# megvii-research/OccDepth

Measured on AMD Instinct MI355X. Metric: frames/sec forward, SemanticKITTI stereo->256x256x32 voxels, higher is better.
Workload: dtype f32 storage and accumulate; matrix arithmetic as 3x bf16 split (hi + mid + lo of both operands, six v_mfma_f32_32x32x16_bf16 per K step; error vs float64 tested within 1.5x of the exact-fp32 kernels', measured 0.8-1.1x) in the head convolutions (K2s3), the small-volume 3x3x3 convolutions and transpo

## Files before the change

include/occdepth_amd.h:

```cpp
#ifndef OCCDEPTH_AMD_H
#define OCCDEPTH_AMD_H

#include <stdint.h>

#ifdef __cplusplus
extern "C" {
#endif

#define OCCD_OK 0
#define OCCD_EINVAL (-1)
#define OCCD_ELAUNCH (-2)
#define OCCD_ENOMEM (-3)

#define OCCD_MAX_VIEWS 4
#define OCCD_MAX_SCALES 4

#define OCCD_ACT_NONE 0
#define OCCD_ACT_RELU 1
#define OCCD_ACT_SIGMOID 2
#define OCCD_ACT_RELU_PRE 3

#define OCCD_ABI_VERSION 22
int occd_abi_version(void);
const char* occd_strerror(int code);
// ... 153 lines not shown
    const double* cam_E;
    const double* cam_k;
    double voxel_size;
    float origin[3];
    int32_t img_w, img_h;
    occd_flosp_args frustum;
    const float* ida;
} occd_lift_proj_args;
int occd_lift_proj_fwd(const occd_lift_proj_args* a, void* stream);

typedef struct occd_lift_bwd_args {
    occd_lift_args fwd;
    const float* gout;
    float* gfeat[OCCD_MAX_SCALES][OCCD_MAX_VIEWS];
    float* gdepth;
} occd_lift_bwd_args;
int occd_lift_bwd(const occd_lift_bwd_args* a, void* stream);

int occd_project_voxels(const double* cam_E_host, const double* cam_k_host, const double* vox_origin_host,
                        double voxel_size, int32_t X, int32_t Y, int32_t Z, int32_t img_w, int32_t img_h,
                        int64_t* pix, uint8_t* fov, float* pix_z, void* stream);

typedef struct occd_vox2pix_args {
    const double* cam_E;
    const double* cam_k;
    const float* ida;
    int64_t* pix;
    uint8_t* fov;
    float* pix_z;
    double vox_origin[3];
    double voxel_size;
    int32_t batch, n_views, X, Y, Z;
    int32_t img_w, img_h;
} occd_vox2pix_args;
int occd_vox2pix(const occd_vox2pix_args* a, void* stream);

int occd_nchw_to_nhwc(const float* in, float* out, int32_t batch, int32_t C,
                      int64_t S, int32_t cs, void* stream);
int occd_nhwc_to_nchw(const float* in, float* out, int32_t batch, int32_t C,
                      int64_t S, int32_t cs, int32_t coff, void* stream);
int occd_softmax_channels(const float* src, float* dst, int64_t rows,
                          int32_t src_cs, int32_t src_coff, int32_t dst_cs,
                          int32_t dst_coff, int32_t n, int32_t dst_pad, void* stream);

int occd_cascade_tail_fwd(const float* part, const float* wn, float* out, int32_t batch, int32_t X,
                          int32_t Y, int32_t Z, int32_t part_cs, int32_t occ_off, int32_t out_cs,
                          int32_t nbr, void* stream);

int occd_affine_act_nchw(const float* x, const float* res, float* y, const float* scale,
                         const float* shift, int32_t batch, int32_t C, int64_t S, int32_t act,
                         float slope, int32_t res_first, void* stream);

int occd_swish_bwd(const float* x, const float* gy, float* gx, int64_t n, void* stream);
int occd_softmax_nchw(const float* x, float* y, int32_t batch, int32_t C, int64_t S, void* stream);
int occd_dwconv2d_nchw(const float* x, const float* w, const float* scale, const float* shift,
                       float* y, int32_t batch, int32_t C, int32_t H, int32_t W, int32_t k,
                       int32_t stride, int32_t pad_top, int32_t pad_left, int32_t Ho, int32_t Wo,
                       int32_t act, void* stream);
int occd_stem_conv3x3_nchw(const float* x, const float* w, const float* scale, const float* shift, float* y,
                           int32_t batch, int32_t H, int32_t W, int32_t cout, int32_t stride, int32_t pad_top,
                           int32_t pad_left, int32_t Ho, int32_t Wo, int32_t act, void* stream);
int occd_upsample_bilinear_cat_nchw(const float* x, const float* skip, float* out, int32_t batch,
                                    int32_t C, int32_t Cskip, int32_t h, int32_t w, int32_t H,
                                    int32_t W, void* stream);
int occd_upsample_bilinear_cat_nhwc(const float* x, const float* skip, float* out, int32_t batch, int32_t C, int32_t Cskip,
                                    int32_t h, int32_t w, int32_t H, int32_t W, void* stream);
int occd_upsample_bilinear_cat_nhwc_rows(const float* x, const float* skip, float* out, int32_t batch, int32_t C, int32_t Cskip,
                                         int32_t h, int32_t w, int32_t H, int32_t W, int32_t out_cs, void* stream);
int occd_upsample_bilinear_nhwc_bwd(const float* gout, float* gx, int32_t batch, int32_t C, int32_t gout_cs, int32_t h,
                                    int32_t w, int32_t H, int32_t W, void* stream);

int occd_upconv_gather_nchw(const float* z, float* out, int32_t batch, int32_t Cout, int32_t h, int32_t w,
                            int32_t H, int32_t W, int64_t z_channel_stride, int64_t z_batch_stride, void* stream);

int occd_upconv_gather_skip_nchw(const float* z, const float* skip, const float* wskip, const float* shift, float* out,
                                 int32_t batch, int32_t Cout, int32_t Cs, int32_t h, int32_t w, int32_t H, int32_t W,
                                 int64_t z_channel_stride, int64_t z_batch_stride, float slope, void* stream);

int occd_wino_input_transform_nchw(const float* x, float* V, int32_t batch, int32_t Cin, int32_t H, int32_t W,
                                   int32_t ty0, int32_t ths, void* stream);
int occd_wino_output_transform_nchw(const float* M, const float* scale, const float* shift, const float* res,
                                    float* y, int32_t batch, int32_t Cout, int32_t H, int32_t W, int32_t ty0,
                                    int32_t ths, int32_t act, float slope, int32_t res_first, void* stream);

typedef struct occd_wino_args {
    const float* x;
    const float* upk;
    const float* shift;
    const float* res;
    float* y;
    int32_t batch, cin, cout, H, W;
    int32_t act, res_first, tile_hint;
    float slope;
} occd_wino_args;
int64_t occd_wino_packed_floats(int32_t cout, int32_t cin);
int occd_wino_pack_weights(const float* w, const float* scale, float* upk, int32_t cout, int32_t cin, void* stream);
int occd_wino_conv3x3_fwd(const occd_wino_args* a, void* stream);

int64_t occd_wino_packed_f16x2_bytes(int32_t cout, int32_t cin);
int occd_wino_pack_weights_f16x2(const float* w, const float* scale, void* upk, int32_t cout, int32_t cin, void* stream);
int occd_wino_conv3x3_f16x2_fwd(const occd_wino_args* a, void* stream);
int occd_wino_conv3x3_f16x2_fwd_ex(const occd_wino_args* a, int32_t max_workgroups, void* stream);

int occd_dwconv2d_bwd_data_nchw(const float* gy, const float* w, float* dx, int32_t batch, int32_t C, int32_t H,
                                int32_t W, int32_t k, int32_t stride, int32_t pad_top, int32_t pad_left, int32_t Ho,
                                int32_t Wo, void* stream);
int64_t occd_dwconv2d_bwd_weight_workspace_floats(int32_t batch, int32_t C, int32_t k, int32_t Ho, int32_t Wo);
int occd_dwconv2d_bwd_weight_nchw(const float* x, const float* gy, float* dw, float* workspace, int32_t batch, int32_t C,
                                  int32_t H, int32_t W, int32_t k, int32_t stride, int32_t pad_top, int32_t pad_left,
                                  int32_t Ho, int32_t Wo, void* stream);
int32_t occd_dwconv2d_pool_blocks(int32_t Ho, int32_t Wo);
int occd_dwconv2d_pool_nchw(const float* x, const float* w, const float* scale, const float* shift, float* y,
                            float* pool_part, int32_t batch, int32_t C, int32_t H, int32_t W, int32_t k,
                            int32_t stride, int32_t pad_top, int32_t pad_left, int32_t Ho, int32_t Wo,
                            int32_t act, int64_t x_plane_stride, void* stream);
int32_t occd_dwconv2d_set_stage(int32_t form);
int occd_plane_reduce(const float* a, const float* b, float* out, int64_t planes, int64_t S, void* stream);
int occd_se_bwd(const float* gg, const float* gate, const float* sums, const float* r, const float* w_reduce,
                const float* b_reduce, const float* w_expand, float* dz_scratch, float* gm, float* gw_reduce,
                float* gb_reduce, float* gw_expand, float* gb_expand, int32_t batch, int32_t C, int32_t Cr, int64_t S,
                void* stream);
int occd_depthnet_gate(const float* sps, const float* intrins, int64_t intr_stride, float factor, const float* w1,
                       const float* b1, const float* w2, const float* b2, const float* wr, const float* br,
                       const float* we, const float* be, float* gate, int32_t images, int32_t C, void* stream);
int occd_se_gate(const float* pool_part, const float* w_reduce, const float* b_reduce, const float* w_expand,
                 const float* b_expand, float* r_scratch, float* gate, int32_t batch, int32_t C, int32_t Cr,
                 int32_t nblk, int64_t S, void* stream);
int32_t occd_se_gate_set_fused(int32_t on);

int occd_graph_replace_memsets(void* graph);

typedef struct occd_pw_args {
    const float* x;
    const float* wpk;
    const float* shift;
    const float* gate;
    const float* res;
    float* y;
    int64_t N;
    int32_t batch, cin, cout;
    int32_t act, tile_hint;
    float slope;
    int32_t out_nhwc_cs;
} occd_pw_args;
int64_t occd_pw_packed_floats(int32_t cout, int32_t cin);
int occd_pw_pack_weights(const float* w, const float* scale, float* wpk, int32_t cout, int32_t cin, void* stream);
int occd_pw_conv_fwd(const occd_pw_args* a, void* stream);

int occd_argmax_channels(const float* x, int64_t rows, int32_t cs, int32_t coff, int32_t C,
                         const uint16_t* lut, uint16_t* out, void* stream);

#define OCCD_RENDER_MAX_VIEWS 8
typedef struct OccdRenderView {
    float o0[3], ou[3], ov[3];
    float d0[3], du[3], dv[3];
} OccdRenderView;

typedef struct OccdRenderArgs {
    const void* labels;
    const void* target;
    const uint8_t* fov;
    const OccdRenderView* views;
    const uint8_t* palette;
    const uint8_t* background;
    uint8_t* rgb;
    int32_t* hit;
// ... 327 lines not shown
```

occdepth_amd/csrc/wino2d.hip:

```cpp
#include "device.h"

namespace {

constexpr int kTilesX = 32;
constexpr int kCh = 32;
constexpr int kCols = 2 * kTilesX + 2;

__global__ void __launch_bounds__(256) wino_input_kernel(const float* __restrict__ x, float* __restrict__ V, int B,
                                                         int Cin, int H, int W, int ths, int tw, int ty0) {
    __shared__ float tile[kCh][4 * kCols + 1];
    const int cblocks = (Cin + kCh - 1) / kCh;
    const int b = blockIdx.z / cblocks, c0 = (blockIdx.z - b * cblocks) * kCh;
    const int tys = blockIdx.y, ty = ty0 + tys, tx0 = blockIdx.x * kTilesX;
    const int y0 = 2 * ty - 1, x0 = 2 * tx0 - 1;
    for (int i = threadIdx.x; i < kCh * 4 * kCols; i += 256) {
        const int col = i % kCols, rc = i / kCols;
        const int r = rc & 3, c = rc >> 2;
        const int yy = y0 + r, xx = x0 + col, cc = c0 + c;
        float v = 0.f;
        if (cc < Cin && yy >= 0 && yy < H && xx >= 0 && xx < W) v = x[(((size_t)b * Cin + cc) * H + yy) * W + xx];
        tile[c][r * kCols + col] = v;
    }
    __syncthreads();
    const int c = threadIdx.x & 31;
// ... 3 lines not shown
        if (tx >= tw || c0 + c >= Cin) continue;
        float d[4][4];
#pragma unroll
        for (int r = 0; r < 4; ++r)
#pragma unroll
            for (int j = 0; j < 4; ++j) d[r][j] = tile[c][r * kCols + 2 * t + j];
        float w[4][4];
#pragma unroll
        for (int j = 0; j < 4; ++j) {
            w[0][j] = d[0][j] - d[2][j];
            w[1][j] = d[1][j] + d[2][j];
            w[2][j] = d[2][j] - d[1][j];
            w[3][j] = d[1][j] - d[3][j];
        }
        const size_t tidx = ((size_t)b * ths + tys) * tw + tx;
        float* o = V + tidx * Cin + c0 + c;
        const size_t xs = T * Cin;
#pragma unroll
        for (int r = 0; r < 4; ++r) {
            o[(size_t)(4 * r + 0) * xs] = w[r][0] - w[r][2];
            o[(size_t)(4 * r + 1) * xs] = w[r][1] + w[r][2];
            o[(size_t)(4 * r + 2) * xs] = w[r][2] - w[r][1];
            o[(size_t)(4 * r + 3) * xs] = w[r][1] - w[r][3];
        }
    }
}

__global__ void __launch_bounds__(256) wino_output_kernel(const float* __restrict__ M, const float* __restrict__ scale,
                                                          const float* __restrict__ shift, const float* __restrict__ res,
                                                          float* __restrict__ y, int B, int Cout, int H, int W, int ths,
                                                          int tw, int ty0, int act, float slope, int res_first) {
    __shared__ float tile[kCh][2 * 2 * kTilesX + 1];
    const int cblocks = (Cout + kCh - 1) / kCh;
    const int b = blockIdx.z / cblocks, c0 = (blockIdx.z - b * cblocks) * kCh;
    const int tys = blockIdx.y, ty = ty0 + tys, tx0 = blockIdx.x * kTilesX;
    const int c = threadIdx.x & 31;
    const size_t T = (size_t)B * ths * tw;
    const size_t xs = T * Cout;
    for (int t = threadIdx.x >> 5; t < kTilesX; t += 8) {
        const int tx = tx0 + t;
        float o[2][2] = {{0.f, 0.f}, {0.f, 0.f}};
        if (tx < tw && c0 + c < Cout) {
            const size_t tidx = ((size_t)b * ths + tys) * tw + tx;
            const float* m = M + tidx * Cout + c0 + c;
            float v[4][4];
#pragma unroll
            for (int r = 0; r < 4; ++r)
#pragma unroll
                for (int j = 0; j < 4; ++j) v[r][j] = m[(size_t)(4 * r + j) * xs];
            float s[2][4];
#pragma unroll
            for (int j = 0; j < 4; ++j) {
                s[0][j] = v[0][j] + v[1][j] + v[2][j];
                s[1][j] = v[1][j] - v[2][j] - v[3][j];
            }
#pragma unroll
            for (int r = 0; r < 2; ++r) {
                o[r][0] = s[r][0] + s[r][1] + s[r][2];
                o[r][1] = s[r][1] - s[r][2] - s[r][3];
            }
        }
#pragma unroll
        for (int r = 0; r < 2; ++r) {
            tile[c][r * 2 * kTilesX + 2 * t] = o[r][0];
            tile[c][r * 2 * kTilesX + 2 * t + 1] = o[r][1];
        }
    }
    __syncthreads();
    for (int i = threadIdx.x; i < kCh * 2 * 2 * kTilesX; i += 256) {
        const int col = i & (2 * kTilesX - 1), rc = i >> 6;
        const int r = rc & 1, cc = rc >> 1;
        const int yy = 2 * ty + r, xx = 2 * tx0 + col, ch = c0 + cc;
        if (ch >= Cout || yy >= H || xx >= W) continue;
        const size_t idx = (((size_t)b * Cout + ch) * H + yy) * W + xx;
        float v = tile[cc][r * 2 * kTilesX + col];
        v = v * (scale != nullptr ? scale[ch] : 1.f) + (shift != nullptr ? shift[ch] : 0.f);
        if (res != nullptr && res_first) v += res[idx];
        v = act2d_exact(v, act, slope);
        if (res != nullptr && !res_first) v += res[idx];
        y[idx] = v;
    }
}

}

extern "C" {

int occd_wino_input_transform_nchw(const float* x, float* V, int32_t batch, int32_t Cin, int32_t H, int32_t W,
                                   int32_t ty0, int32_t ths, void* stream) {
    if (!x || !V || batch <= 0 || Cin <= 0 || H <= 0 || W <= 0) return OCCD_EINVAL;
    const int tw = (W + 1) / 2;
    if (ty0 < 0 || ths < 1 || ty0 + ths > (H + 1) / 2) return OCCD_EINVAL;
    const int th = ths;
    const long gz = (long)batch * ((Cin + kCh - 1) / kCh);
    if (gz > 65535 || th > 65535) return OCCD_EINVAL;
    const double T = (double)batch * th * tw;
    occd::ProfScope prof("wino_input", (hipStream_t)stream, 32.0 * T * Cin, 4.0 * ((double)batch * Cin * H * W + 16.0 * T * Cin));
    hipLaunchKernelGGL(wino_input_kernel, dim3((unsigned)((tw + kTilesX - 1) / kTilesX), (unsigned)th, (unsigned)gz), dim3(256),
                       0, (hipStream_t)stream, x, V, batch, Cin, H, W, ths, tw, ty0);
    return occd::check_launch();
}

int occd_wino_output_transform_nchw(const float* M, const float* scale, const float* shift, const float* res, float* y,
                                    int32_t batch, int32_t Cout, int32_t H, int32_t W, int32_t ty0, int32_t ths,
                                    int32_t act, float slope, int32_t res_first, void* stream) {
    if (!M || !y || batch <= 0 || Cout <= 0 || H <= 0 || W <= 0 || act < 0 || act > 3) return OCCD_EINVAL;
    const int tw = (W + 1) / 2;
    if (ty0 < 0 || ths < 1 || ty0 + ths > (H + 1) / 2) return OCCD_EINVAL;
    const int th = ths;
    const long gz = (long)batch * ((Cout + kCh - 1) / kCh);
    if (gz > 65535 || th > 65535) return OCCD_EINVAL;
    const double T = (double)batch * th * tw;
    occd::ProfScope prof("wino_output", (hipStream_t)stream, 24.0 * T * Cout,
                         4.0 * (16.0 * T * Cout + (double)batch * Cout * H * W * (1 + (res != nullptr))));
    hipLaunchKernelGGL(wino_output_kernel, dim3((unsigned)((tw + kTilesX - 1) / kTilesX), (unsigned)th, (unsigned)gz), dim3(256),
                       0, (hipStream_t)stream, M, scale, shift, res, y, batch, Cout, H, W, ths, tw, ty0, act, slope, res_first);
    return occd::check_launch();
}

}
```

occdepth_amd/hip.py:

```python
import ctypes
import os
from ctypes import c_int32, c_int64, c_void_p

import torch

from . import abi

_HERE = os.path.dirname(os.path.abspath(__file__))
LIB_PATH = os.path.join(_HERE, "libocc_hip.so")

EXPORTS = abi.EXPORTS
ABI_VERSION = abi.ABI_VERSION
MAX_VIEWS = abi.CONSTANTS["OCCD_MAX_VIEWS"]
MAX_SCALES = abi.CONSTANTS["OCCD_MAX_SCALES"]
ACT_NONE = abi.CONSTANTS["OCCD_ACT_NONE"]
ACT_RELU = abi.CONSTANTS["OCCD_ACT_RELU"]
ACT_SIGMOID = abi.CONSTANTS["OCCD_ACT_SIGMOID"]
ACT_RELU_PRE = abi.CONSTANTS["OCCD_ACT_RELU_PRE"]
OPTIM_CHUNK = abi.CONSTANTS["OCCD_OPTIM_CHUNK"]
MAX_REGIONS = abi.CONSTANTS["OCCD_MAX_REGIONS"]

Conv3dArgs = abi.STRUCTS["occd_conv3d_args"]
WgradArgs = abi.STRUCTS["occd_conv3d_wgrad_args"]
FlospArgs = abi.STRUCTS["occd_flosp_args"]
# ... 560 lines not shown
        ctx.save_for_backward(xc, w)
        ctx.plain = bool(autograd3d.BF16_MFMA) and PW_TRAIN == "bf16"
        return gemm_x3(w.detach().reshape(w.shape[0], C), xc.view(B, C, H * W), plain_bf16=ctx.plain).view(B, w.shape[0], H, W)

    @staticmethod
    @torch.amp.custom_bwd(device_type="cuda")
    def backward(ctx, gy):
        x, w = ctx.saved_tensors
        B, C, H, W = x.shape
        Co = w.shape[0]
        g = gy.float()
        g = (g if g.is_contiguous() else g.contiguous()).view(B, Co, H * W)
        gx = gw = None
        if ctx.needs_input_grad[0]:
            gx = gemm_x3(w.detach().reshape(Co, C).t().contiguous(), g, plain_bf16=ctx.plain).view(B, C, H, W)
        if ctx.needs_input_grad[1]:
            gw = gemm_x3_nt(g, x.view(B, C, H * W), plain_bf16=ctx.plain).view(Co, C, 1, 1)
        return gx, gw


PW_TRAIN = os.environ.get("OCCDEPTH_TRAIN_PW_GEMM", "1")


def pw_conv_autograd_ok(conv, x):
    if PW_TRAIN not in ("1", "bf16"):
        return False
    dt_ok = x.dtype == torch.float32 or (torch.is_autocast_enabled() and x.dtype in (torch.bfloat16, torch.float16))
    return (GEMM_X3 and x.is_cuda and x.dim() == 4 and dt_ok
            and conv.kernel_size == (1, 1) and conv.stride == (1, 1) and conv.groups == 1 and conv.bias is None
            and conv.dilation == (1, 1) and conv.in_channels % 8 == 0 and conv.out_channels % 8 == 0
            and x.shape[2] * x.shape[3] >= 4 and x.shape[0] <= 65535)


def pw_conv_autograd(x, w):
    return _PwConvFn.apply(x, w)


GEMM_X3 = os.environ.get("OCCDEPTH_GEMM_X3", "1") == "1"


GEMM_X3_PACK = os.environ.get("OCCDEPTH_GEMM_X3_PACK", "0") == "1"


GEMM_X3_PANEL = os.environ.get("OCCDEPTH_GEMM_X3_PANEL", "1") == "1"
PANEL_MAX_K, PANEL_MIN_ROWS = 848, 256


def _panel_operand(w, role):
    return GEMM_X3_PANEL and role == "a" and w.dim() == 2 and w.shape[0] >= PANEL_MIN_ROWS


def _panel_launch(pa, b):
    if pa.K <= 352:
        return True
    if pa.K > PANEL_MAX_K:
        return False
    n, batch = b.shape[-1], (b.shape[0] if b.dim() == 3 else 1)
    return -(-n // 64) * batch * -(-(-(-pa.rows // 32)) // 8) <= 512


def _presplit_launch(pa, b):
    n, batch = b.shape[-1], (b.shape[0] if b.dim() == 3 else 1)
    return pa.K >= 512 and -(-pa.rows // 256) * -(-n // 128) * batch >= 320


def gemm_split():
    from . import fused
    return fused.GEMM_SPLIT


def set_gemm_split(v):
    from . import fused
    fused.set_gemm_split(v)


SPLITK_F16X2_MIN_TILE_STEPS = 140


def splitk_f16x2_wins(M, N, K, batch):
    per, _, rr, _ = gemm_x3_splitk_plan(M, N, K, batch)
    return -(-(-(-M // 32)) // rr) * per >= SPLITK_F16X2_MIN_TILE_STEPS


def gemm_packed_a(w, split):
    if split == "f16x2":
        try:
            return GemmPacked(w, "a", split="f16x2")
        except ValueError:
            pass
    return GemmPacked(w, "a")


def matmul_operand(w, role, split=None):
    w = w.detach().float().contiguous()
    if GEMM_X3 and w.is_cuda and (GEMM_X3_PACK or _panel_operand(w, role)):
        return w, (gemm_packed_a(w, split) if split is not None and role == "a" else GemmPacked(w, role))
    return w, None


PAD_ROWS = os.environ.get("OCCDEPTH_PAD_ROWS", "1") == "1"


def padded_rows(shape, device):
    n = int(shape[-1])
    pitch = round_up(n, 32) if PAD_ROWS else n
    return torch.empty(tuple(shape[:-1]) + (pitch,), device=device, dtype=torch.float32)[..., :n]


def matmul(a, b, bias=None, act=None, slope=0.01, res=None, k_scale=None, out=None):
    ta, pa = a if isinstance(a, tuple) else (a, None)
    tb, pb = b if isinstance(b, tuple) else (b, None)
    if GEMM_X3:
        a_img = pa is not None and (GEMM_X3_PACK or (res is None and k_scale is None and
                                                     (_panel_launch(pa, tb) or _presplit_launch(pa, tb))))
        xa, xb = (pa if a_img else ta), (pb if pb is not None and k_scale is None else tb)
        if gemm_x3_supported(xa, xb):
            return gemm_x3(xa, xb, bias=bias, act=act, slope=slope, res=res, k_scale=k_scale, out=out)
        if gemm_x3_supported(ta, tb):
            return gemm_x3(ta, tb, bias=bias, act=act, slope=slope, res=res, k_scale=k_scale, out=out)
    if k_scale is not None:
        tb = tb * k_scale.unsqueeze(-1)
    y = torch.matmul(ta, tb)
    if bias is not None:
        y = y + bias.view(-1, 1)
    if act == "swish":
        y = y * torch.sigmoid(y)
    elif act == "leaky":
        y = torch.nn.functional.leaky_relu(y, slope)
    y = y + res if res is not None else y
    if out is not None:
        out.copy_(y)
        return out
    return y


def c32x3_eligible(x, cout, kernel, out, stride=(1, 1, 1), dilation=(1, 1, 1), padding=(0, 0, 0), res1=None, res2=None,
                   act_in=ACT_NONE, act_out=ACT_NONE, out_pos=None, o_stride=(1, 1, 1), o_off=(0, 0, 0), cin=None,
                   tile_hint=0):
    d = tuple(dilation)
    if tuple(kernel) != (3, 3, 3) or tuple(stride) != (1, 1, 1) or d[0] != d[1] or d[0] != d[2] or not 1 <= d[0] <= 3:
        return False
    if tuple(padding) != d or (out_pos is not None and tuple(out_pos) != tuple(x.dims)) or tuple(o_stride) != (1, 1, 1) or \
            tuple(o_off) != (0, 0, 0):
        return False
    c = x.C if cin is None else cin
    if round_up(c, 8) != 32 or cout > 32 or x.coff + 32 > x.cs or act_in == ACT_SIGMOID or tile_hint != 0:
        return False
    if x.buf.dtype != torch.float32 or x.cs % 4 or x.coff % 4:
        return False
    X, Y, Z = x.dims
    if Z % 32 or tuple(out.dims) != (X, Y, Z):
        return False
    return x.batch * X * ((Y + 7) // 8) * (Z // 32) >= 512 and x.batch * X * Y * Z * x.cs < 2 ** 32


_wgrad_ws = {}


def conv3d_wgrad(x, gy, cin, cout, kernel, stride=(1, 1, 1), dilation=(1, 1, 1), padding=(0, 0, 0)):
    a = WgradArgs()
    a.x, a.gy = _f32(x.buf, "x"), _f32(gy.buf, "gy")
    a.batch = x.batch
    a.X, a.Y, a.Z = x.dims
    a.cin, a.x_cs, a.x_coff = cin, x.cs, x.coff
    a.Xo, a.Yo, a.Zo = gy.dims
    a.cout, a.gy_cs, a.gy_coff = cout, gy.cs, gy.coff
    a.kx, a.ky, a.kz = kernel
    a.sx, a.sy, a.sz = stride
    a.dx, a.dy, a.dz = dilation
    a.px, a.py, a.pz = padding
    need = load().occd_conv3d_wgrad_workspace_floats(ctypes.byref(a))
    if need <= 0:
        raise RuntimeError(f"occd_conv3d_wgrad_workspace_floats failed (code {need})")
    dev = x.buf.device
    ws = _wgrad_ws.get(dev)
    if ws is None or ws.numel() < need:
        ws = torch.empty(need, dtype=torch.float32, device=dev)
        _wgrad_ws[dev] = ws
    dw = torch.empty((cout, cin) + tuple(kernel), dtype=torch.float32, device=dev)
    a.dw, a.workspace, a.workspace_floats = dw.data_ptr(), ws.data_ptr(), ws.numel()
    if _PROFILING:
        set_tag("%d>%d k%d%d%d s%d%d%d d%d%d%d @%dx%dx%d" % ((cin, cout) + tuple(kernel) + tuple(stride)
                                                              + tuple(dilation) + tuple(x.dims)))
    _check(load().occd_conv3d_wgrad(ctypes.byref(a), _stream()), "occd_conv3d_wgrad")
    return dw


def conv3d_wgrad_bf16(x, gy, cin, cout, kernel, stride=(1, 1, 1), dilation=(1, 1, 1), padding=(0, 0, 0)):
    code = _storage_code(x.buf.dtype)
    ptr = _act_ptr(x.buf.dtype)
    a = WgradArgs()
    a.x, a.gy = ptr(x.buf, "x"), ptr(gy.buf, "gy")
    a.batch = x.batch
    a.X, a.Y, a.Z = x.dims
    a.cin, a.x_cs, a.x_coff = cin, x.cs, x.coff
    a.Xo, a.Yo, a.Zo = gy.dims
    a.cout, a.gy_cs, a.gy_coff = cout, gy.cs, gy.coff
# ... 238 lines not shown
    out = torch.empty((B,) + sp + (cs,), device=x.device, dtype=torch.float32)
    xc = x.contiguous()
    _check(load().occd_nchw_to_nhwc(_f32(xc, "x"), _f32(out, "out"), B, C, S, cs, _stream()), "occd_nchw_to_nhwc")
    return out


def nhwc_to_nchw(vox):
    B = vox.batch
    X, Y, Z = vox.dims
    out = torch.empty((B, vox.C, X, Y, Z), device=vox.buf.device, dtype=torch.float32)
    _check(load().occd_nhwc_to_nchw(_f32(vox.buf, "in"), _f32(out, "out"), B, vox.C, X * Y * Z, vox.cs, vox.coff,
                                    _stream()), "occd_nhwc_to_nchw")
    return out


def softmax_channels(src, dst, n, dst_pad=0):
    rows = src.batch * src.dims[0] * src.dims[1] * src.dims[2]
    if _PROFILING:
        set_tag("%d @%d rows" % (n, rows))
    _check(load().occd_softmax_channels(_f32(src.buf, "src"), _f32(dst.buf, "dst"), rows, src.cs, src.coff, dst.cs,
                                        dst.coff, n, dst_pad, _stream()), "occd_softmax_channels")
    return dst


ACT2D = {None: 0, "none": 0, "relu": 1, "swish": 2, "leaky": 3}


def affine_act(x, scale, shift, act=None, slope=0.01, res=None, res_first=False, out=None):
    if not x.is_contiguous():
        x = x.contiguous()
    B, C = x.shape[0], x.shape[1]
    S = x.numel() // (B * C)
    out = x if out is None else out
    if res is not None and not res.is_contiguous():
        res = res.contiguous()
    if _PROFILING:
        set_tag("%d @%dx%d" % (C, B, S))
    _check(load().occd_affine_act_nchw(_f32(x, "x"), _f32(res, "res") if res is not None else None, _f32(out, "out"),
                                       _f32(scale, "scale") if scale is not None else None,
                                       _f32(shift, "shift") if shift is not None else None, B, C, S, ACT2D[act],
                                       float(slope), 1 if res_first else 0, _stream()), "occd_affine_act_nchw")
    return out


_WINO_G = ((1.0, 0.0, 0.0), (0.5, 0.5, 0.5), (0.5, -0.5, 0.5), (0.0, 0.0, 1.0))


def winograd_weights(w):
    G = torch.tensor(_WINO_G, dtype=torch.float64, device=w.device)
    u = torch.einsum("ia,ocab,jb->ijco", G, w.detach().double(), G)
    return u.reshape(16, w.shape[1], w.shape[0]).float().contiguous()


def wino_input_transform(x, ty0=0, ths=None):
    B, C, H, W = x.shape
    ths = (H + 1) // 2 - ty0 if ths is None else ths
    T = B * ths * ((W + 1) // 2)
    V = torch.empty((16, T, C), device=x.device, dtype=torch.float32)
    xc = x if x.is_contiguous() else x.contiguous()
    if _PROFILING:
        set_tag("%d @%dx%dx%d" % (C, B, H, W))
    _check(load().occd_wino_input_transform_nchw(_f32(xc, "x"), V.data_ptr(), B, C, H, W, ty0, ths, _stream()),
           "occd_wino_input_transform_nchw")
    return V


def wino_output_transform(M, shape, scale=None, shift=None, act=None, slope=0.01, res=None, res_first=False, out=None,
                          ty0=0, ths=None):
    B, C, H, W = shape
    ths = (H + 1) // 2 - ty0 if ths is None else ths
    y = torch.empty(shape, device=M.device, dtype=torch.float32) if out is None else out
    if res is not None and not res.is_contiguous():
        res = res.contiguous()
    if _PROFILING:
        set_tag("%d @%dx%dx%d" % (C, B, H, W))
    _check(load().occd_wino_output_transform_nchw(_f32(M, "M"), _f32(scale, "scale") if scale is not None else None,
                                                  _f32(shift, "shift") if shift is not None else None,
                                                  _f32(res, "res") if res is not None else None, _f32(y, "y"), B, C, H, W,
                                                  ty0, ths, ACT2D[act], float(slope), 1 if res_first else 0, _stream()),
           "occd_wino_output_transform_nchw")
    return y


def conv2d_3x3_winograd(x, U, scale=None, shift=None, act=None, slope=0.01, res=None, res_first=False, strip_rows=None):
    B, Cin, H, W = x.shape
    cout = (U[0] if isinstance(U, tuple) else U).shape[2]
    th = (H + 1) // 2
    if strip_rows is None or strip_rows >= th:
        V = wino_input_transform(x)
        return wino_output_transform(matmul(V, U), (B, cout, H, W), scale, shift, act, slope, res, res_first)
    y = torch.empty((B, cout, H, W), device=x.device, dtype=torch.float32)
    xc = x if x.is_contiguous() else x.contiguous()
    for ty0 in range(0, th, strip_rows):
        ths = min(strip_rows, th - ty0)
        M = matmul(wino_input_transform(xc, ty0, ths), U)
        wino_output_transform(M, tuple(y.shape), scale, shift, act, slope, res, res_first, out=y, ty0=ty0, ths=ths)
    return y


def wino_pack_weights(w, scale=None):
    cout, cin = w.shape[0], w.shape[1]
    if tuple(w.shape[2:]) != (3, 3):
        raise RuntimeError("wino_pack_weights needs a (Cout, Cin, 3, 3) weight")
    n = load().occd_wino_packed_floats(cout, cin)
    if n <= 0:
        raise RuntimeError("occd_wino_packed_floats: bad shape")
    wc = w.detach().float().contiguous()
    upk = torch.empty(n, device=w.device, dtype=torch.float32)
    sc = scale.detach().float().contiguous() if scale is not None else None
    _check(load().occd_wino_pack_weights(_f32(wc, "w"), _f32(sc, "scale") if sc is not None else None,
                                         _f32(upk, "upk"), cout, cin, _stream()), "occd_wino_pack_weights")
    return upk


class WinoF16x2:

    __slots__ = ("image", "cout", "cin", "f32")

    def __init__(self, image, cout, cin, f32=None):
        self.image, self.cout, self.cin, self.f32 = image, cout, cin, f32


_CU_COUNT = {}


def _cu_count(device):
    n = _CU_COUNT.get(device)
    if n is None:
        n = _CU_COUNT[device] = torch.cuda.get_device_properties(device).multi_processor_count
    return n


def wino_f16x2_wins(B, cin, cout, H, W, device=None):
    tiles = B * ((H + 1) // 2) * ((W + 1) // 2)
    return ((cout + 31) // 32) * ((tiles + 127) // 128) >= _cu_count(torch.cuda.current_device() if device is None else device)


def wino_pack_weights_f16x2(w, scale=None):
    cout, cin = w.shape[0], w.shape[1]
    if tuple(w.shape[2:]) != (3, 3):
        raise RuntimeError("wino_pack_weights_f16x2 needs a (Cout, Cin, 3, 3) weight")
    n = load().occd_wino_packed_f16x2_bytes(cout, cin)
    if n <= 0:
        raise RuntimeError("occd_wino_packed_f16x2_bytes: bad shape")
    wc = w.detach().float().contiguous()
    sc = scale.detach().float().contiguous() if scale is not None else None
    image = torch.empty(n, device=w.device, dtype=torch.uint8)
    rc = load().occd_wino_pack_weights_f16x2(_f32(wc, "w"), _f32(sc, "scale") if sc is not None else None,
                                             _ptr(image, "upk"), cout, cin, _stream())
    if rc == -1:
        raise ValueError("wino_pack_weights_f16x2: non-finite weights (keep the float32 image of wino_pack_weights)")
    _check(rc, "occd_wino_pack_weights_f16x2")
    return WinoF16x2(image, cout, cin)


def _parse_wino_persist(value):
    if value not in ("0", "1"):
        raise ValueError("OCCDEPTH_WINO_PERSIST must be 0 or 1, not %r" % (value,))
    return value == "1"


WINO_PERSIST = _parse_wino_persist(os.environ.get("OCCDEPTH_WINO_PERSIST", "0"))


def conv2d_3x3_fused(x, upk, cout, shift=None, act=None, slope=0.01, res=None, res_first=False, tile_hint=0, out=None,
                     max_workgroups=None):
    if not x.is_contiguous():
        x = x.contiguous()
    B, cin, H, W = x.shape
    y = torch.empty((B, cout, H, W), device=x.device, dtype=torch.float32) if out is None else out
# ... 1121 lines not shown
```

occdepth_amd/models/efficientnet.py:

```python
import math

import torch
import torch.nn as nn
import torch.nn.functional as F

import os

from .. import hip
from .. import fused as _fused
from ..bn import bn_act
from ..fused import _stamp, bn_affine_cached, needs_autograd

PW_FUSED = os.environ.get("OCCDEPTH_PW_FUSED", "1") == "1"
PW_MIN_PIXELS = int(os.environ.get("OCCDEPTH_PW_MIN_PIXELS", "0"))


def pw_wins(x):
    return PW_FUSED and x.shape[0] * x.shape[2] * x.shape[3] >= PW_MIN_PIXELS


PW_EXPAND_LIB_BELOW = int(os.environ.get("OCCDEPTH_PW_EXPAND_LIB_BELOW", str(1 << 40)))
PW_PLAIN_LIB_BELOW = 14000


def expand_on_library(x):
    below = PW_EXPAND_LIB_BELOW if hip.GEMM_X3 else min(PW_EXPAND_LIB_BELOW, PW_PLAIN_LIB_BELOW)
    return x.shape[1] % 8 == 0 and x.shape[0] * x.shape[2] * x.shape[3] < below


def pw_operands(owner, conv, bn=None):
    key = _stamp(conv, bn)
    cache = owner.__dict__.setdefault("_pw_cache", {})
    hit = cache.get(id(conv))
    if hit is None or hit[0] != key:
        scale = shift = None
        if bn is not None:
            scale, shift = bn_affine_cached(bn)
        if conv.bias is not None:
            b = conv.bias.detach().float()
            shift = b * scale + shift if bn is not None else b
        hit = (key, hip.pw_pack_weights(conv.weight, scale), shift.contiguous() if shift is not None else None)
        cache[id(conv)] = hit
    return hit[1], hit[2]


def gemm_operands(owner, conv, bn):
    key = (_stamp(conv, bn), hip.gemm_split())
    cache = owner.__dict__.setdefault("_gemm_cache", {})
    hit = cache.get(id(conv))
    if hit is None or hit[0] != key:
        scale, shift = bn_affine_cached(bn)
        w = conv.weight.detach().float().flatten(1) * scale.view(-1, 1)
        if conv.bias is not None:
            shift = conv.bias.detach().float() * scale + shift
        hit = (key, hip.matmul_operand(w, "a", split=key[1]), shift.contiguous())
        cache[id(conv)] = hit
    return hit[1], hit[2]


def expand_gemm(owner, conv, bn, x, act, pad_out=False):
    B, C, H, W = x.shape
    if hip.GEMM_X3 and C % 8 == 0 and H * W >= 4 and x.is_contiguous():
        w, shift = gemm_operands(owner, conv, bn)
        out = hip.padded_rows((B, w[0].shape[0], H * W), x.device) if pad_out else None
        return hip.matmul(w, x.view(B, C, H * W), bias=shift, act=act, out=out).view(B, -1, H, W)
    return hip.affine_act(F.conv2d(x, conv.weight), *bn_affine_cached(bn), act)


PW_PROJECT_K16 = os.environ.get("OCCDEPTH_PW_PROJECT_K16", "1") == "1"
PW_PROJECT_K16_MIN_PIXELS = int(os.environ.get("OCCDEPTH_PW_PROJECT_K16_MIN_PIXELS", "3000"))
PW_PROJECT_K16_MIN_COUT = int(os.environ.get("OCCDEPTH_PW_PROJECT_K16_MIN_COUT", "48"))


PW_PROJECT_SPLITK = os.environ.get("OCCDEPTH_PW_PROJECT_SPLITK", "1") == "1"
PW_PROJECT_SPLITK_MIN_K = int(os.environ.get("OCCDEPTH_PW_PROJECT_SPLITK_MIN_K", "768"))
PW_PROJECT_SPLITK_MAX_PIXELS = int(os.environ.get("OCCDEPTH_PW_PROJECT_SPLITK_MAX_PIXELS", "8000"))


def splitk_operands(owner, conv, bn, pixels=None, batch=1):
    split = hip.gemm_split()
    if split == "f16x2" and pixels is not None and not hip.splitk_f16x2_wins(conv.out_channels, pixels, conv.in_channels, batch):
        split = "bf16x3"
    key = (_stamp(conv, bn), split)
    cache = owner.__dict__.setdefault("_splitk_cache", {})
    hit = cache.get(id(conv))
    if hit is None or hit[0] != key:
        scale, shift = bn_affine_cached(bn)
        w = (conv.weight.detach().float().flatten(1) * scale.view(-1, 1)).contiguous()
        if conv.bias is not None:
            shift = conv.bias.detach().float() * scale + shift
        hit = (key, hip.gemm_packed_a(w, key[1]), shift.contiguous())
        cache[id(conv)] = hit
    return hit[1], hit[2]


def project_conv(owner, conv, bn, y, gate, res):
    B, C, H, W = y.shape
    cout = conv.out_channels
    if (PW_PROJECT_SPLITK and hip.GEMM_X3 and y.is_cuda and C % 8 == 0 and C >= PW_PROJECT_SPLITK_MIN_K and H * W >= 4
            and B * H * W <= PW_PROJECT_SPLITK_MAX_PIXELS and y.is_contiguous() and gate.is_contiguous()
            and tuple(gate.shape) == (B, C) and (res is None or res.is_contiguous())):
        pa, shift = splitk_operands(owner, conv, bn, H * W, B)
        out = hip.gemm_x3_splitk(pa, y.view(B, C, H * W), bias=shift, k_scale=gate,
                                 res=res.view(B, cout, H * W) if res is not None else None)
        return out.view(B, cout, H, W)
    if (PW_PROJECT_K16 and hip.GEMM_X3 and C % 8 == 0 and B * H * W >= PW_PROJECT_K16_MIN_PIXELS and y.is_contiguous()
            and cout >= PW_PROJECT_K16_MIN_COUT and gate.is_contiguous() and tuple(gate.shape) == (B, C) and (res is None or res.is_contiguous())):
        w, shift = gemm_operands(owner, conv, bn)
        out = hip.matmul(w, y.view(B, C, H * W), bias=shift, k_scale=gate,
                         res=res.view(B, cout, H * W) if res is not None else None)
        return out.view(B, cout, H, W)
    wpk, shift = pw_operands(owner, conv, bn)
    return hip.conv1x1(y, wpk, cout, shift, None, gate=gate, res=res)


def _fast(x, module):
    return _fused.on_gpu(x) and not needs_autograd(module) and x.dtype == torch.float32

_B0_STAGES = (("ds", 1, 3, 1, 1, 16), ("ir", 2, 3, 2, 6, 24), ("ir", 2, 5, 2, 6, 40), ("ir", 3, 3, 2, 6, 80),
              ("ir", 3, 5, 1, 6, 112), ("ir", 4, 5, 2, 6, 192), ("ir", 1, 3, 1, 6, 320))
_SCALING = {"tf_efficientnet_b3_ns": (1.2, 1.4), "tf_efficientnet_b4_ns": (1.4, 1.8),
            "tf_efficientnet_b5_ns": (1.6, 2.2), "tf_efficientnet_b7_ns": (2.0, 3.1)}
_BN_EPS = 1e-3


def _round_channels(ch, mult, divisor=8):
    ch = ch * mult
    new = max(int(ch + divisor / 2) // divisor * divisor, divisor)
    return new + divisor if new < 0.9 * ch else new


class Conv2dSame(nn.Conv2d):

    def forward(self, x):
        if (self.kernel_size == (1, 1) and self.stride == (1, 1) and self.groups == 1 and _fast(x, self) and pw_wins(x)
                and x.shape[0] * x.shape[2] * x.shape[3] >= PW_PLAIN_LIB_BELOW):
            wpk, shift = pw_operands(self, self)
            return hip.conv1x1(x, wpk, self.out_channels, shift)
# ... 145 lines not shown
```

occdepth_amd/models/unet2d.py:

```python
import os

import torch
import torch.nn as nn
import torch.nn.functional as F

from .. import autograd3d as _ag
from .. import hip
from .. import fused as _fused
from ..fused import _stamp, bn_affine_cached, needs_autograd, wino_fused_operands
from .efficientnet import EfficientNet, pw_operands, pw_wins

MODEL_NAME = "tf_efficientnet_b3_ns"
MODEL_CHANNELS = {
    "tf_efficientnet_b3_ns": [3, 24, 32, 48, 136],
    "tf_efficientnet_b4_ns": [3, 24, 32, 56, 160],
    "tf_efficientnet_b5_ns": [3, 32, 40, 64, 176],
    "tf_efficientnet_b7_ns": [3, 32, 48, 80, 224],
}
NUM_FEATURES = {
    "tf_efficientnet_b3_ns": 1536,
    "tf_efficientnet_b4_ns": 1792,
    "tf_efficientnet_b5_ns": 2048,
    "tf_efficientnet_b7_ns": 2560,
}
_SCALES = (16, 8, 4, 2, 1)


class UpSampleBN(nn.Module):
    def __init__(self, skip_input, output_features):
        super().__init__()
        layers = []
        for cin in (skip_input, output_features):
            layers += [nn.Conv2d(cin, output_features, kernel_size=3, stride=1, padding=1),
                       nn.BatchNorm2d(output_features), nn.LeakyReLU()]
        self._net = nn.Sequential(*layers)

    WINOGRAD = os.environ.get("OCCDEPTH_WINOGRAD", "1") == "1"
    WINOGRAD_MAX_PIXELS = int(os.environ.get("OCCDEPTH_WINOGRAD_MAX_PIXELS", "80000"))
    WINOGRAD_MIN_CIN = int(os.environ.get("OCCDEPTH_WINOGRAD_MIN_CIN", "256"))

    def _wino_operands(self, conv, bn):
        key = _stamp(conv, bn)
        cache = self.__dict__.setdefault("_wino_cache", {})
        hit = cache.get(id(conv))
        if hit is None or hit[0] != key:
            scale, shift = bn_affine_cached(bn)
            if conv.bias is not None:
                shift = shift + scale * conv.bias.detach().float()
            hit = (key, hip.matmul_operand(hip.winograd_weights(conv.weight), "b"), scale.contiguous(), shift.contiguous())
            cache[id(conv)] = hit
        return hit[1:]

    WINOGRAD_HIRES_PIXELS = int(os.environ.get("OCCDEPTH_WINOGRAD_HIRES_PIXELS", "0"))
    WINOGRAD_HIRES_MIN_CIN = int(os.environ.get("OCCDEPTH_WINOGRAD_HIRES_MIN_CIN", "64"))
    WINOGRAD_STRIP_MB = float(os.environ.get("OCCDEPTH_WINOGRAD_STRIP_MB", "96"))

    FUSED_MIN_PIXELS = int(os.environ.get("OCCDEPTH_WINO_FUSED_MIN_PIXELS", "50000"))
    FUSED = os.environ.get("OCCDEPTH_WINO_FUSED", "1") == "1"

    def _fused_operands(self, conv, bn):
        return wino_fused_operands(self, conv, bn)

    TRAIN_K10 = os.environ.get("OCCDEPTH_TRAIN_K10", "1") == "1"

    def _conv_bn_act(self, f, conv, bn, act):
        B, C, H, W = f.shape
        if self.FUSED and B * H * W >= self.FUSED_MIN_PIXELS:
            upk, shift = self._fused_operands(conv, bn)
            return hip.conv2d_3x3_fused(f, upk, conv.out_channels, shift, "leaky", act.negative_slope)
        if self.WINOGRAD and C >= self.WINOGRAD_MIN_CIN and B * H * W <= self.WINOGRAD_MAX_PIXELS:
            U, scale, shift = self._wino_operands(conv, bn)
            return hip.conv2d_3x3_winograd(f, U, scale, shift, "leaky", act.negative_slope)
        if self.WINOGRAD and C >= self.WINOGRAD_HIRES_MIN_CIN and B * H * W <= self.WINOGRAD_HIRES_PIXELS:
            U, scale, shift = self._wino_operands(conv, bn)
            per_row = 16.0 * B * ((W + 1) // 2) * (C + conv.out_channels) * 4
            rows = max(1, int(self.WINOGRAD_STRIP_MB * 2 ** 20 / per_row))
            return hip.conv2d_3x3_winograd(f, U, scale, shift, "leaky", act.negative_slope, strip_rows=rows)
        return hip.affine_act(conv(f), *bn_affine_cached(bn), "leaky", slope=act.negative_slope)

    UPCONV = os.environ.get("OCCDEPTH_UPCONV", "1") == "1"
    UPCONV_LIB_BELOW = int(os.environ.get("OCCDEPTH_UPCONV_LIB_BELOW", str(1 << 62)))
    UPCONV_FOLD_BELOW = int(os.environ.get("OCCDEPTH_UPCONV_FOLD_BELOW", "0"))
    UPCONV_FUSE_SKIP = os.environ.get("OCCDEPTH_UPCONV_FUSE_SKIP", "1") == "1"

    def _upconv_operands(self, conv, bn, cup):
        key = (_stamp(conv, bn), cup, _fused.WINO_SPLIT, hip.gemm_split())
        hit = self.__dict__.get("_upconv_cache")
        if hit is None or hit[0] != key:
            scale, shift = bn_affine_cached(bn)
            if conv.bias is not None:
                shift = shift + scale * conv.bias.detach().float()
            w = conv.weight.detach().float()
            cout = w.shape[0]
            w9 = (w[:, :cup] * scale.view(-1, 1, 1, 1)).permute(2, 3, 0, 1).reshape(9 * cout, cup).contiguous()
            wskip = (w[:, cup:] * scale.view(-1, 1, 1, 1)).contiguous()
            hit = (key, hip.pw_pack_weights(w9), hip.matmul_operand(w9, "a", split=key[3]),
                   _fused.wino_pack(w[:, cup:].contiguous(), scale), shift.contiguous(), wskip)
            self.__dict__["_upconv_cache"] = hit
        return hit[1:]

    @staticmethod
    def _tap_planes(shape, device):
        return hip.padded_rows(shape, device) if hip.GEMM_X3 else None

    def _first_conv_upconv(self, x, skip, conv, bn, act):
        wpk9, w9, upk_skip, shift, wskip = self._upconv_operands(conv, bn, x.shape[1])
        cout = conv.out_channels
        B, cup, h, w = x.shape
        if B > 1 and B * h * w <= self.UPCONV_FOLD_BELOW:
            z = hip.matmul(w9, x.permute(1, 0, 2, 3).reshape(cup, B * h * w),
                           out=self._tap_planes((9 * cout, B * h * w), x.device)).view(9 * cout, B, h, w)
            batch_inner = True
        else:
            batch_inner = False
            if B * h * w < self.UPCONV_LIB_BELOW:
                xc = x if x.is_contiguous() else x.contiguous()
                z = hip.matmul(w9, xc.view(B, cup, h * w), out=self._tap_planes((B, 9 * cout, h * w), x.device)).view(B, 9 * cout, h, w)
            else:
                z = hip.conv1x1(x, wpk9, 9 * cout)
        rw = (w - 1) / max(skip.shape[3] - 1, 1)
        if self.UPCONV_FUSE_SKIP and skip.shape[1] <= 4 and rw * 258.0 + 3.0 <= 191.0:
            return hip.upconv_gather(z, cout, skip.shape[2:], batch_inner=batch_inner, skip=skip, wskip=wskip, shift=shift,
                                     slope=act.negative_slope)
        u = hip.upconv_gather(z, cout, skip.shape[2:], batch_inner=batch_inner)
        return hip.conv2d_3x3_fused(skip, upk_skip, cout, shift, "leaky", act.negative_slope, res=u, res_first=True)

    def _forward_train_cl(self, x, concat_with):
        from ..bn import bn_act
        n = self._net
        if x.dtype == torch.float32 and concat_with.dtype == torch.float32:
            f = hip.upsample_bilinear_cat_cl_autograd(x, concat_with)
        else:
# ... 190 lines not shown
```

Before: 69.39.

## Add channel-major Winograd path with packed-A f16x2 GEMM and small-weight tile GEMM

Adds channel-major Winograd input and output transform kernels so the transformed weights act as the packed A operand (16 x Cout x Cin, f16x2 split) and the transformed input as B. This lets the low-resolution UNet decoder 3x3 convolutions with large Cin run through the packed-A GEMM path, writing M^T directly and fusing BN, activation and residual in the output transform. A second change lets small pointwise weights (fewer rows than the panel threshold) use a prepacked f16x2 A image when the problem is large enough. The cost is extra weight packing, lazily built legacy operands and more dispatch heuristics.

Result: faster. 71.19 (median of 6 runs) (+2.6%).

```diff
diff --git a/include/occdepth_amd.h b/include/occdepth_amd.h
--- a/include/occdepth_amd.h
+++ b/include/occdepth_amd.h
@@ -259,6 +259,12 @@
 int occd_wino_output_transform_nchw(const float* M, const float* scale, const float* shift, const float* res,
                                     float* y, int32_t batch, int32_t Cout, int32_t H, int32_t W, int32_t ty0,
                                     int32_t ths, int32_t act, float slope, int32_t res_first, void* stream);
+
+int occd_wino_input_transform_cm(const float* x, float* Vt, int32_t batch, int32_t Cin, int32_t H, int32_t W,
+                                 int64_t Tp, void* stream);
+int occd_wino_output_transform_cm(const float* Mt, const float* scale, const float* shift, const float* res,
+                                  float* y, int32_t batch, int32_t Cout, int32_t H, int32_t W, int64_t Tp,
+                                  int32_t act, float slope, int32_t res_first, void* stream);
 
 typedef struct occd_wino_args {
     const float* x;
diff --git a/occdepth_amd/csrc/wino2d.hip b/occdepth_amd/csrc/wino2d.hip
--- a/occdepth_amd/csrc/wino2d.hip
+++ b/occdepth_amd/csrc/wino2d.hip
@@ -109,9 +109,167 @@
     }
 }
 
+constexpr int kCmCh = 4;
+
+struct __attribute__((packed, aligned(4))) F4u { float v[4]; };
+struct __attribute__((packed, aligned(4))) F2u { float v[2]; };
+
+__global__ void __launch_bounds__(256) wino_input_cm_kernel(const float* __restrict__ x, float* __restrict__ Vt, int Cin, int H,
+                                                            int W, int th, int tw, long T, long Tp) {
+    const long t = (long)blockIdx.x * 256 + threadIdx.x;
+    if (t >= T) return;
+    const int tx = (int)(t % tw);
+    const long q = t / tw;
+    const int ty = (int)(q % th), b = (int)(q / th);
+    const int y0 = 2 * ty - 1, x0 = 2 * tx - 1;
+    const int xc = min(max(x0, 0), W - 4), sh = x0 - xc;
+    const size_t xs = (size_t)Cin * Tp;
+#pragma unroll
+    for (int cc = 0; cc < kCmCh; ++cc) {
+        const int c = blockIdx.y * kCmCh + cc;
+        if (c >= Cin) break;
+        const float* xp = x + ((size_t)b * Cin + c) * H * W;
+        float d[4][4];
+#pragma unroll
+        for (int r = 0; r < 4; ++r) {
+            const int yy = y0 + r;
+            const bool row = yy >= 0 && yy < H;
+            const float* rp = xp + (size_t)min(max(yy, 0), H - 1) * W;
+            if (W >= 4) {
+                const F4u p = *reinterpret_cast<const F4u*>(rp + xc);
+#pragma unroll
+                for (int j = 0; j < 4; ++j) {
+                    const int s = j + sh;
+                    const float v = s == 0 ? p.v[0] : s == 1 ? p.v[1] : s == 2 ? p.v[2] : s == 3 ? p.v[3] : 0.f;
+                    d[r][j] = row ? v : 0.f;
+                }
+            } else {
+#pragma unroll
+                for (int j = 0; j < 4; ++j) {
+                    const int xx = x0 + j;
+                    const float v = rp[min(max(xx, 0), W - 1)];
+                    d[r][j] = row && xx >= 0 && xx < W ? v : 0.f;
+                }
+            }
+        }
+        float w[4][4];
+#pragma unroll
+        for (int j = 0; j < 4; ++j) {
+            w[0][j] = d[0][j] - d[2][j];
+            w[1][j] = d[1][j] + d[2][j];
+            w[2][j] = d[2][j] - d[1][j];
+            w[3][j] = d[1][j] - d[3][j];
+        }
+        float* o = Vt + (size_t)c * Tp + t;
+#pragma unroll
+        for (int r = 0; r < 4; ++r) {
+            o[(size_t)(4 * r + 0) * xs] = w[r][0] - w[r][2];
+            o[(size_t)(4 * r + 1) * xs] = w[r][1] + w[r][2];
+            o[(size_t)(4 * r + 2) * xs] = w[r][2] - w[r][1];
+            o[(size_t)(4 * r + 3) * xs] = w[r][1] - w[r][3];
+        }
+    }
+}
+
+__global__ void __launch_bounds__(256) wino_output_cm_kernel(const float* __restrict__ Mt, const float* __restrict__ scale,
+                                                             const float* __restrict__ shift, const float* __restrict__ res,
+                                                             float* __restrict__ y, int Cout, int H, int W, int th, int tw,
+                                                             long T, long Tp, int act, float slope, int res_first) {
+    const long t = (long)blockIdx.x * 256 + threadIdx.x;
+    if (t >= T) return;
+    const int tx = (int)(t % tw);
+    const long q = t / tw;
+    const int ty = (int)(q % th), b = (int)(q / th);
+    const int xx = 2 * tx;
+    const bool pair = xx + 1 < W;
+    const size_t xs = (size_t)Cout * Tp;
+#pragma unroll
+    for (int cc = 0; cc < kCmCh; ++cc) {
+        const int ch = blockIdx.y * kCmCh + cc;
+        if (ch >= Cout) break;
+        const float* m = Mt + (size_t)ch * Tp + t;
+        float v[4][4];
+#pragma unroll
+        for (int r = 0; r < 4; ++r)
+#pragma unroll
+            for (int j = 0; j < 4; ++j) v[r][j] = m[(size_t)(4 * r + j) * xs];
+        float s[2][4];
+#pragma unroll
+        for (int j = 0; j < 4; ++j) {
+            s[0][j] = v[0][j] + v[1][j] + v[2][j];
+            s[1][j] = v[1][j] - v[2][j] - v[3][j];
+        }
+        float o[2][2];
+#pragma unroll
+        for (int r = 0; r < 2; ++r) {
+            o[r][0] = s[r][0] + s[r][1] + s[r][2];
+            o[r][1] = s[r][1] - s[r][2] - s[r][3];
+        }
+        const float sc = scale != nullptr ? scale[ch] : 1.f, sh = shift != nullptr ? shift[ch] : 0.f;
+#pragma unroll
+        for (int r = 0; r < 2; ++r) {
+            const int yy = 2 * ty + r;
+            if (yy >= H) continue;
+            const size_t idx = (((size_t)b * Cout + ch) * H + yy) * W + xx;
+            float rv[2] = {0.f, 0.f};
+            if (res != nullptr) {
+                if (pair) {
+                    const F2u p = *reinterpret_cast<const F2u*>(res + idx);
+                    rv[0] = p.v[0]; rv[1] = p.v[1];
+                } else {
+                    rv[0] = res[idx];
+                }
+            }
+            F2u out;
+#pragma unroll
+            for (int j = 0; j < 2; ++j) {
+                float u = o[r][j];
+                u = u * sc + sh;
+                if (res != nullptr && res_first) u += rv[j];
+                u = act2d_exact(u, act, slope);
+                if (res != nullptr && !res_first) u += rv[j];
+                out.v[j] = u;
+            }
+            if (pair) *reinterpret_cast<F2u*>(y + idx) = out;
+            else y[idx] = out.v[0];
+        }
+    }
+}
+
+inline bool wino_cm_geometry(int32_t batch, int32_t C, int32_t H, int32_t W, int64_t Tp, long* T, long* gx, long* gy) {
+    if (batch <= 0 || C <= 0 || H <= 0 || W <= 0) return false;
+    *T = (long)batch * ((H + 1) / 2) * ((W + 1) / 2);
+    if (Tp < *T || (Tp & 31)) return false;
+    *gx = (*T + 255) / 256;
+    *gy = ((long)C + kCmCh - 1) / kCmCh;
+    return *gx < (1L << 31) && *gy <= 65535;
+}
+
 }
 
 extern "C" {
+
+int occd_wino_input_transform_cm(const float* x, float* Vt, int32_t batch, int32_t Cin, int32_t H, int32_t W, int64_t Tp,
+                                 void* stream) {
+    long T, gx, gy;
+    if (!x || !Vt || !wino_cm_geometry(batch, Cin, H, W, Tp, &T, &gx, &gy)) return OCCD_EINVAL;
+    occd::ProfScope prof("wino_input_cm", (hipStream_t)stream, 32.0 * T * Cin, 4.0 * ((double)batch * Cin * H * W + 16.0 * T * Cin));
+    hipLaunchKernelGGL(wino_input_cm_kernel, dim3((unsigned)gx, (unsigned)gy), dim3(256), 0, (hipStream_t)stream, x, Vt, Cin, H, W,
+                       (H + 1) / 2, (W + 1) / 2, T, (long)Tp);
+    return occd::check_launch();
+}
+
+int occd_wino_output_transform_cm(const float* Mt, const float* scale, const float* shift, const float* res, float* y,
+                                  int32_t batch, int32_t Cout, int32_t H, int32_t W, int64_t Tp, int32_t act, float slope,
+                                  int32_t res_first, void* stream) {
+    long T, gx, gy;
+    if (!Mt || !y || act < 0 || act > 3 || !wino_cm_geometry(batch, Cout, H, W, Tp, &T, &gx, &gy)) return OCCD_EINVAL;
+    occd::ProfScope prof("wino_output_cm", (hipStream_t)stream, 24.0 * T * Cout,
+                         4.0 * (16.0 * T * Cout + (double)batch * Cout * H * W * (1 + (res != nullptr))));
+    hipLaunchKernelGGL(wino_output_cm_kernel, dim3((unsigned)gx, (unsigned)gy), dim3(256), 0, (hipStream_t)stream, Mt, scale, shift,
+                       res, y, Cout, H, W, (H + 1) / 2, (W + 1) / 2, T, (long)Tp, act, slope, res_first);
+    return occd::check_launch();
+}
 
 int occd_wino_input_transform_nchw(const float* x, float* V, int32_t batch, int32_t Cin, int32_t H, int32_t W,
                                    int32_t ty0, int32_t ths, void* stream) {
diff --git a/occdepth_amd/hip.py b/occdepth_amd/hip.py
--- a/occdepth_amd/hip.py
+++ b/occdepth_amd/hip.py
@@ -666,6 +666,14 @@
     return -(-(-(-M // 32)) // rr) * per >= SPLITK_F16X2_MIN_TILE_STEPS
 
 
+TILE_F16X2 = os.environ.get("OCCDEPTH_GEMM_TILE_F16X2", "1") == "1"
+TILE_F16X2_MIN_ROWS, TILE_F16X2_MIN_COLS = 48, 3000
+
+
+def tile_f16x2_wins(M, N, K, batch):
+    return TILE_F16X2 and M >= TILE_F16X2_MIN_ROWS and N * batch >= TILE_F16X2_MIN_COLS
+
+
 def gemm_packed_a(w, split):
     if split == "f16x2":
         try:
@@ -675,10 +683,15 @@
     return GemmPacked(w, "a")
 
 
-def matmul_operand(w, role, split=None):
+def matmul_operand(w, role, split=None, small=False):
     w = w.detach().float().contiguous()
     if GEMM_X3 and w.is_cuda and (GEMM_X3_PACK or _panel_operand(w, role)):
         return w, (gemm_packed_a(w, split) if split is not None and role == "a" else GemmPacked(w, role))
+    if GEMM_X3 and w.is_cuda and small and split == "f16x2" and role == "a" and w.dim() == 2 and GEMM_X3_PANEL:
+        try:
+            return w, GemmPacked(w, "a", split="f16x2")
+        except ValueError:
+            pass
     return w, None
 
 
@@ -695,8 +708,12 @@
     ta, pa = a if isinstance(a, tuple) else (a, None)
     tb, pb = b if isinstance(b, tuple) else (b, None)
     if GEMM_X3:
-        a_img = pa is not None and (GEMM_X3_PACK or (res is None and k_scale is None and
-                                                     (_panel_launch(pa, tb) or _presplit_launch(pa, tb))))
+        if pa is not None and pa.rows < PANEL_MIN_ROWS and not GEMM_X3_PACK:
+            n, batch = tb.shape[-1], (tb.shape[0] if tb.dim() == 3 else 1)
+            a_img = pa.split == "f16x2" and tile_f16x2_wins(pa.rows, n, pa.K, batch)
+        else:
+            a_img = pa is not None and (GEMM_X3_PACK or (res is None and k_scale is None and
+                                                         (_panel_launch(pa, tb) or _presplit_launch(pa, tb))))
         xa, xb = (pa if a_img else ta), (pb if pb is not None and k_scale is None else tb)
         if gemm_x3_supported(xa, xb):
             return gemm_x3(xa, xb, bias=bias, act=act, slope=slope, res=res, k_scale=k_scale, out=out)
@@ -1101,10 +1118,78 @@
     return y
 
 
-def conv2d_3x3_winograd(x, U, scale=None, shift=None, act=None, slope=0.01, res=None, res_first=False, strip_rows=None):
+class WinoCM:
+
+    def __init__(self, w, make_u):
+        self.cout, self.cin = int(w.shape[0]), int(w.shape[1])
+        ut = winograd_weights(w).transpose(1, 2).contiguous()
+        self.image = GemmPacked(ut, "a", split="f16x2")
+        self._make_u, self._u = make_u, None
+
+    def u(self):
+        if self._u is None:
+            self._u = self._make_u()
+        return self._u
+
+
+WINO_CM = os.environ.get("OCCDEPTH_WINO_CM", "1") == "1"
+WINO_CM_MIN_CIN, WINO_CM_MIN_WORKGROUPS = 512, 320
+
+
+def wino_cm_wins(B, cin, cout, H, W):
+    T = B * ((H + 1) // 2) * ((W + 1) // 2)
+    return WINO_CM and cin >= WINO_CM_MIN_CIN and cin % 8 == 0 and T >= 4 and \
+        16 * -(-cout // 256) * -(-T // 128) >= WINO_CM_MIN_WORKGROUPS
+
+
+def wino_input_transform_cm(x, Tp=None):
+    B, C, H, W = x.shape
+    T = B * ((H + 1) // 2) * ((W + 1) // 2)
+    Tp = round_up(T, 32) if Tp is None else Tp
+    Vt = torch.empty((16, C, Tp), device=x.device, dtype=torch.float32)
+    xc = x if x.is_contiguous() else x.contiguous()
+    if _PROFILING:
+        set_tag("%d @%dx%dx%d" % (C, B, H, W))
+    _check(load().occd_wino_input_transform_cm(_f32(xc, "x"), Vt.data_ptr(), B, C, H, W, Tp, _stream()),
+           "occd_wino_input_transform_cm")
+    return Vt[..., :T]
+
+
+def wino_output_transform_cm(Mt, shape, scale=None, shift=None, act=None, slope=0.01, res=None, res_first=False):
+    B, C, H, W = shape
+    T = B * ((H + 1) // 2) * ((W + 1) // 2)
+    if Mt.dtype != torch.float32 or tuple(Mt.shape) != (16, C, T) or Mt.stride(2) != 1 or Mt.stride(0) != C * Mt.stride(1):
+        raise RuntimeError("wino_output_transform_cm: M^T must be (16, C, T) float32 over dense padded rows")
+    y = torch.empty(shape, device=Mt.device, dtype=torch.float32)
+    if res is not None and not res.is_contiguous():
+        res = res.contiguous()
+    if _PROFILING:
+        set_tag("%d @%dx%dx%d" % (C, B, H, W))
+    if not Mt.is_cuda or Mt.stride(1) < T or Mt.stride(1) % 32:
+        raise RuntimeError("wino_output_transform_cm: M^T must be a GPU tensor with rows on a pitch of 32 floats")
+    _check(load().occd_wino_output_transform_cm(Mt.data_ptr(), _f32(scale, "scale") if scale is not None else None,
+                                                _f32(shift, "shift") if shift is not None else None,
+                                                _f32(res, "res") if res is not None else None, _f32(y, "y"), B, C, H, W,
+                                                Mt.stride(1), ACT2D[act], float(slope), 1 if res_first else 0, _stream()),
+           "occd_wino_output_transform_cm")
+    return y
+
+
+def conv2d_3x3_winograd(x, U, scale=None, shift=None, act=None, slope=0.01, res=None, res_first=False, strip_rows=None,
+                        cm=None):
     B, Cin, H, W = x.shape
+    th = (H + 1) // 2
+    if isinstance(U, WinoCM):
+        whole = strip_rows is None or strip_rows >= th
+        if GEMM_X3 and whole and x.is_cuda and (wino_cm_wins(B, Cin, U.cout, H, W) if cm is None else cm):
+            if U.cin != Cin:
+                raise RuntimeError("conv2d_3x3_winograd: the WinoCM operand does not match the input channels")
+            Vt = wino_input_transform_cm(x)
+            Mt = torch.empty((16, U.cout, Vt.stride(1)), device=x.device, dtype=torch.float32)[..., :Vt.shape[2]]
+            gemm_x3(U.image, Vt, out=Mt)
+            return wino_output_transform_cm(Mt, (B, U.cout, H, W), scale, shift, act, slope, res, res_first)
+        U = U.u()
     cout = (U[0] if isinstance(U, tuple) else U).shape[2]
-    th = (H + 1) // 2
     if strip_rows is None or strip_rows >= th:
         V = wino_input_transform(x)
         return wino_output_transform(matmul(V, U), (B, cout, H, W), scale, shift, act, slope, res, res_first)
diff --git a/occdepth_amd/models/efficientnet.py b/occdepth_amd/models/efficientnet.py
--- a/occdepth_amd/models/efficientnet.py
+++ b/occdepth_amd/models/efficientnet.py
@@ -53,7 +53,7 @@
         w = conv.weight.detach().float().flatten(1) * scale.view(-1, 1)
         if conv.bias is not None:
             shift = conv.bias.detach().float() * scale + shift
-        hit = (key, hip.matmul_operand(w, "a", split=key[1]), shift.contiguous())
+        hit = (key, hip.matmul_operand(w, "a", split=key[1], small=True), shift.contiguous())
         cache[id(conv)] = hit
     return hit[1], hit[2]
 
diff --git a/occdepth_amd/models/unet2d.py b/occdepth_amd/models/unet2d.py
--- a/occdepth_amd/models/unet2d.py
+++ b/occdepth_amd/models/unet2d.py
@@ -40,14 +40,24 @@
     WINOGRAD_MIN_CIN = int(os.environ.get("OCCDEPTH_WINOGRAD_MIN_CIN", "256"))
 
     def _wino_operands(self, conv, bn):
-        key = _stamp(conv, bn)
+        key = (_stamp(conv, bn), hip.gemm_split())
         cache = self.__dict__.setdefault("_wino_cache", {})
         hit = cache.get(id(conv))
         if hit is None or hit[0] != key:
             scale, shift = bn_affine_cached(bn)
             if conv.bias is not None:
                 shift = shift + scale * conv.bias.detach().float()
-            hit = (key, hip.matmul_operand(hip.winograd_weights(conv.weight), "b"), scale.contiguous(), shift.contiguous())
+
+            def make_u():
+                return hip.matmul_operand(hip.winograd_weights(conv.weight), "b")
+
+            U = None
+            if key[1] == "f16x2" and hip.GEMM_X3 and conv.weight.is_cuda:
+                try:
+                    U = hip.WinoCM(conv.weight.detach().float(), make_u)
+                except ValueError:
+                    pass
+            hit = (key, make_u() if U is None else U, scale.contiguous(), shift.contiguous())
             cache[id(conv)] = hit
         return hit[1:]
 
```
